# translearn/PaintRL

Measured on NVIDIA B200. Metric: batched env steps/sec, higher is better.
Workload: dtype f64

## Files before the change

### paintrl_b200/csrc/paintrl_kernels.cuh

```cuda
#pragma once
#include "paintrl_device.cuh"

namespace paintrl {

struct StepIO {
    const void *actions;
    double *obs, *reward, *penalty, *actual;
    uint8_t *done;
    int32_t *new_texels;
    double *next_obs;
    const int32_t *reset_start_idx;
};

struct EnvSel {
    const int32_t *ids;
    int lo, n;
};

template <bool SUBSET>
__device__ __forceinline__ bool step_env(const EnvSel &sel, int k, int num_envs, int &env) {
    if (!SUBSET) { env = k; return k < num_envs; }
    if (k >= sel.n) return false;
    env = sel.ids ? __ldg(&sel.ids[k]) : sel.lo + k;
    return (unsigned)env < (unsigned)num_envs;
}

struct EnvArrays {
    EnvState *states;
    MoveOut *moves;
    EnvStat *env_stats;
    unsigned *bits;
    int16_t *thick;
    unsigned *grid_cnt;
    unsigned *ready;
    ShotPoses *shots;
    unsigned *last_mask;
};

constexpr int kStageWords = 512;

template <bool STAGED>
struct alignas(128) WarpScratch {
    unsigned sbits[STAGED ? kStageWords : 32];
    EnvState st;
    MoveOut mv;
    int rowL[kMaxRows], rowU[kMaxRows];
    int rowWa[kMaxRows], rowWn[kMaxRows];
    uint16_t cand[STAGED ? kStageWords : 2];
    double hsi_r[2 * kPaintPerAction];
    unsigned long long bar;
};
static_assert(2 * kMaxRows >= 2 * kMaxObs, "the section histogram aliases rowWa / rowWn");

template <bool STAGED>
struct Bits {
    unsigned *g;
    unsigned *s;
    __device__ __forceinline__ unsigned ld(int w) const { return STAGED ? s[w] : __ldcg(g + w); }
    __device__ __forceinline__ void st(int w, unsigned v) const {
        if (STAGED) s[w] = v; else __stcg(g + w, v);
    }
};

__device__ __forceinline__ unsigned smem_addr(const void *p) { return (unsigned)__cvta_generic_to_shared(p); }
__device__ __forceinline__ void mbar_init(unsigned long long *bar, int count) {
    asm volatile("mbarrier.init.shared::cta.b64 [%0], %1;" ::"r"(smem_addr(bar)), "r"(count) : "memory");
    asm volatile("fence.proxy.async.shared::cta;" ::: "memory");
}
__device__ __forceinline__ void mbar_expect_tx(unsigned long long *bar, unsigned bytes) {
    asm volatile("mbarrier.arrive.expect_tx.shared::cta.b64 _, [%0], %1;" ::"r"(smem_addr(bar)), "r"(bytes) : "memory");
}
__device__ __forceinline__ void bulk_g2s(void *dst, const void *src, unsigned bytes, unsigned long long *bar) {
    asm volatile("cp.async.bulk.shared::cluster.global.mbarrier::complete_tx::bytes [%0], [%1], %2, [%3];" ::"r"(smem_addr(dst)),
                 "l"(src), "r"(bytes), "r"(smem_addr(bar))
                 : "memory");
}
__device__ __forceinline__ void mbar_wait(unsigned long long *bar, unsigned phase) {
    asm volatile(
        "{\n"
        ".reg .pred p;\n"
        "WAIT_%=:\n"
        "mbarrier.try_wait.parity.shared::cta.b64 p, [%0], %1;\n"
        "@p bra DONE_%=;\n"
        "bra WAIT_%=;\n"
        "DONE_%=:\n"
        "}" ::"r"(smem_addr(bar)), "r"(phase)
        : "memory");
}
__device__ __forceinline__ void bulk_s2g(void *dst, const void *src, unsigned bytes) {
    asm volatile("cp.async.bulk.global.shared::cta.bulk_group [%0], [%1], %2;" ::"l"(dst), "r"(smem_addr(src)), "r"(bytes)
                 : "memory");
    asm volatile("cp.async.bulk.commit_group;" ::: "memory");
}
__device__ __forceinline__ void bulk_wait_read() { asm volatile("cp.async.bulk.wait_group.read 0;" ::: "memory"); }
__device__ __forceinline__ void fence_async_smem() { asm volatile("fence.proxy.async.shared::cta;" ::: "memory"); }

__device__ __forceinline__ unsigned lowmask(int n) {
    unsigned m;
    asm("bmsk.clamp.b32 %0, 0, %1;" : "=r"(m) : "r"(n));
    return m;
}
__device__ __forceinline__ int clamp32(int v) { return max(v, 0); }

__device__ __forceinline__ unsigned *bits_of(const DevPack &pk, const EnvArrays &ea, int env) {
    return ea.bits + (size_t)env * pk.n_words_pad;
}
__device__ __forceinline__ int16_t *thick_of(const DevPack &pk, const EnvArrays &ea, int env) {
    return ea.thick ? ea.thick + (size_t)env * pk.n_slots : nullptr;
}
__device__ __forceinline__ unsigned *grid_cnt_of(const DevPack &pk, const EnvArrays &ea, int env) {
    return ea.grid_cnt ? ea.grid_cnt + (size_t)env * pk.n_gcells_pad : nullptr;
}
__device__ __forceinline__ const double *axis_table(const DevPack &pk, int a) {
    return a == 0 ? pk.tx : (a == 1 ? pk.ty : pk.tz);
}

template <typename WS>
__device__ __forceinline__ void row_ranks(const DevPack &pk, const Ax &ax, double p0, int lane, WS &ws) {
    const double f = floor((p0 - pk.cx_o0) * pk.cx_inv);
    const double *kx = axis_table(pk, ax.a0);
    for (int r = lane; r < pk.n_rows; r += 32) {
        const int n = __ldg(&pk.row_count[r]);
        int L, U;
        if (!(f >= 0.0)) {
            L = U = 0;
        } else if (f >= (double)pk.ncx) {
            L = U = n;
        } else {
// ... 228 lines not shown
    const double2 *src = reinterpret_cast<const double2 *>(&st);
    double2 v = src[0];
#pragma unroll
    for (int i = 1; i < 8; ++i) if (lane == i) v = src[i];
    if (lane < 8) reinterpret_cast<double2 *>(g)[lane] = v;
}

__device__ __forceinline__ int auto_start_index(const DevPack &pk, const DevConfig &cfg, int env, int episode) {
    return (int)(splitmix64(cfg.seed ^ splitmix64(((unsigned long long)env << 32) | (unsigned)episode)) %
                 (unsigned long long)pk.n_starts);
}

constexpr float kBallEps = 1e-7f;
constexpr int NS = kPaintPerAction;

struct ShotsF { float x[NS + 1], y[NS + 1], z[NS + 1]; };

template <typename WS>
__device__ __forceinline__ double cen(const WS &ws, int s, int k) {
    return s < NS ? ws.mv.centers[s][k] : ws.st.last_center[k];
}

__device__ __forceinline__ bool ball_pretest_at(const ShotsF &c, float tx, float ty, float tz, float e[NS + 1]) {
    const float nr2f = -(float)(kPaintRadius * kPaintRadius);
    float m = INFINITY;
#pragma unroll
    for (int s = 0; s <= NS; ++s) {
        const float dx = tx - c.x[s], dy = ty - c.y[s], dz = tz - c.z[s];
        e[s] = fmaf(dz, dz, fmaf(dy, dy, fmaf(dx, dx, nr2f)));
        m = fminf(m, fabsf(e[s]));
    }
    return m <= kBallEps;
}
__device__ __forceinline__ bool ball_pretest(const DevPack &pk, const ShotsF &c, int j, float e[NS + 1]) {
    return ball_pretest_at(c, __ldg(&pk.fx[j]), __ldg(&pk.fy[j]), __ldg(&pk.fz[j]), e);
}

template <typename WS>
__device__ __forceinline__ bool ball_exact(const WS &ws, double x, double y, double z, int s) {
    const double r2 = kPaintRadius * kPaintRadius;
    const double dx = x - cen(ws, s, 0), dy = y - cen(ws, s, 1), dz = z - cen(ws, s, 2);
    return (dx * dx + dy * dy + dz * dz) <= r2;
}

template <typename WS>
__device__ __forceinline__ unsigned ball_mask(const DevPack &pk, const ShotsF &c, const WS &ws, int j, bool has_last) {
    float e[NS + 1];
    unsigned in = 0;
    if (ball_pretest(pk, c, j, e)) {
        const double x = __ldg(&pk.tx[j]), y = __ldg(&pk.ty[j]), z = __ldg(&pk.tz[j]);
#pragma unroll
        for (int s = 0; s <= NS; ++s) in |= (ball_exact(ws, x, y, z, s) ? 1u : 0u) << s;
    } else {
#pragma unroll
        for (int s = 0; s <= NS; ++s) in |= (e[s] <= 0.f ? 1u : 0u) << s;
    }
    if (!has_last) in &= (1u << NS) - 1u;
    return in;
}

template <typename WS>
__device__ __forceinline__ void ball_flags_at(const DevPack &pk, const ShotsF &c, const WS &ws, int j, float tx, float ty, float tz,
                                              bool has_last, bool &any_shot, bool &possible) {
    float e[NS + 1];
    bool in[NS + 1];
    if (ball_pretest_at(c, tx, ty, tz, e)) {
        const double x = __ldg(&pk.tx[j]), y = __ldg(&pk.ty[j]), z = __ldg(&pk.tz[j]);
#pragma unroll
        for (int s = 0; s <= NS; ++s) in[s] = ball_exact(ws, x, y, z, s);
    } else {
#pragma unroll
        for (int s = 0; s <= NS; ++s) in[s] = e[s] <= 0.f;
    }
    bool prev = has_last && in[NS];
    any_shot = false;
    possible = false;
#pragma unroll
    for (int s = 0; s < NS; ++s) {
        any_shot = any_shot || in[s];
        possible = possible || (in[s] && !prev);
        prev = in[s];
    }
}
template <typename WS>
__device__ __forceinline__ void ball_flags(const DevPack &pk, const ShotsF &c, const WS &ws, int j, bool has_last, bool &any_shot,
                                           bool &possible) {
    ball_flags_at(pk, c, ws, j, __ldg(&pk.fx[j]), __ldg(&pk.fy[j]), __ldg(&pk.fz[j]), has_last, any_shot, possible);
}

template <bool STAGED, int COLOR, typename WS>
__device__ __forceinline__ int stamp_ranges(const DevPack &pk, float lo0, float hi0, float lo1, float hi1, int lane, WS &ws) {
    const float rr = (float)kPaintRadius + 4e-5f;
    int base = 0;
    for (int r0 = 0; r0 < pk.n_rows; r0 += 32) {
        const int r = r0 + lane;
        int wa = 0, wn = 0;
        if (r < pk.n_rows) {
            const float ylo = fmaf((float)r, pk.rel_row_h, pk.rel_row_o1) - 2e-5f, yhi = ylo + pk.rel_row_h + 4e-5f;
            const float dy = fmaxf(0.f, fmaxf(ylo - hi1, lo1 - yhi));
            if (dy <= rr) {
                const float hw = sqrtf(rr * rr - dy * dy) + 4e-5f;
                const float fa = floorf((lo0 - hw - pk.rel_cx_o0) * pk.rel_cx_inv) - 1.f;
                const float fb = floorf((hi0 + hw - pk.rel_cx_o0) * pk.rel_cx_inv) + 1.f;
                if (fb >= 0.f && fa < (float)pk.ncx) {
                    const int ca = (int)fmaxf(fa, 0.f), cb = (int)fminf(fb, (float)(pk.ncx - 1));
                    const int *cs = pk.cell_start + (size_t)r * (pk.ncx + 1);
                    const int i0 = __ldg(cs + ca), i1 = __ldg(cs + cb + 1);
                    if (i1 > i0) {
                        wa = __ldg(&pk.row_word0[r]) + (i0 >> 5);
                        wn = ((i1 - 1) >> 5) - (i0 >> 5) + 1;
                    }
                }
            }
            ws.rowWa[r] = wa;
            ws.rowWn[r] = wn;
        }
        if (STAGED) {
            int incl = wn;
#pragma unroll
            for (int o = 1; o < 32; o <<= 1) {
                const int u = __shfl_up_sync(kFull, incl, o);
                if (lane >= o) incl += u;
            }
            const int at = base + incl - wn;
            for (int t = 0; t < wn; ++t) ws.cand[at + t] = (uint16_t)(wa + t);
            base += __shfl_sync(kFull, incl, 31);
        }
    }
    __syncwarp();
    return base;
}

template <bool STAGED, typename WS, typename BodyFn>
__device__ __forceinline__ void for_each_stamp_word(const DevPack &pk, int lane, const WS &ws, int n_cand, BodyFn body) {
    if constexpr (STAGED) {
        for (int k = 0; k < n_cand; ++k) body((int)ws.cand[k]);
    } else {
        for (int r0 = 0; r0 < pk.n_rows; r0 += 32) {
            const int r = r0 + lane;
            const int wa = r < pk.n_rows ? ws.rowWa[r] : 0, wn = r < pk.n_rows ? ws.rowWn[r] : 0;
            unsigned m = __ballot_sync(kFull, wn > 0);
            while (m) {
                const int src = __ffs(m) - 1;
                m &= m - 1;
                const int a = __shfl_sync(kFull, wa, src), n = __shfl_sync(kFull, wn, src);
                for (int w = a; w < a + n; ++w) body(w);
            }
        }
    }
}

template <int COLOR, bool STAGED, typename WS, typename BITS>
__device__ __forceinline__ void stamp(const DevPack &pk, const Ax &ax, const BITS &bits, int16_t *thick, unsigned *grid_cnt, bool has_last,
                                      int lane, WS &ws, int &n_new_out, int &n_possible_out, bool &dirty_out PAINTRL_PROF_PARAM) {
    ShotsF c;
#pragma unroll
    for (int s = 0; s <= NS; ++s) {
        c.x[s] = (float)(cen(ws, s, 0) - pk.org0);
        c.y[s] = (float)(cen(ws, s, 1) - pk.org1);
        c.z[s] = (float)(cen(ws, s, 2) - pk.org2);
    }
    float lo0 = INFINITY, hi0 = -INFINITY, lo1 = INFINITY, hi1 = -INFINITY;
#pragma unroll
    for (int s = 0; s < NS; ++s) {
        const float c0 = ax.a0 == 0 ? c.x[s] : (ax.a0 == 1 ? c.y[s] : c.z[s]);
        const float c1 = ax.a1 == 0 ? c.x[s] : (ax.a1 == 1 ? c.y[s] : c.z[s]);
        lo0 = fminf(lo0, c0); hi0 = fmaxf(hi0, c0);
        lo1 = fminf(lo1, c1); hi1 = fmaxf(hi1, c1);
    }
    PAINTRL_PROF(17, lane == 0);
    const int n_cand = stamp_ranges<STAGED, COLOR>(pk, lo0, hi0, lo1, hi1, lane, ws);
    PAINTRL_PROF(18, lane == 0);

    double rmax[NS];
    if (COLOR == 1) {
#pragma unroll
        for (int s = 0; s < NS; ++s) rmax[s] = -1.0;
        for_each_stamp_word<STAGED>(pk, lane, ws, n_cand, [&](int w) {
            const int j = w * 32 + lane;
            const unsigned in = ball_mask(pk, c, ws, j, false);
            if (in) {
                const double x = __ldg(&pk.tx[j]), y = __ldg(&pk.ty[j]), z = __ldg(&pk.tz[j]);
#pragma unroll
                for (int s = 0; s < NS; ++s) {
                    if (in & (1u << s)) {
                        const double dx = x - cen(ws, s, 0), dy = y - cen(ws, s, 1), dz = z - cen(ws, s, 2);
                        rmax[s] = fmax(rmax[s], dx * dx + dy * dy + dz * dz);
                    }
                }
            }
        });
#pragma unroll
        for (int s = 0; s < NS; ++s) rmax[s] = sqrt(warp_max(rmax[s]));
        if (lane < NS) {
            double r = rmax[0];
#pragma unroll
            for (int s = 1; s < NS; ++s) r = lane == s ? rmax[s] : r;
            ws.hsi_r[lane] = r;
            ws.hsi_r[NS + lane] = r > 0.0 ? 1.0 / (r * r) : 0.0;
        }
        __syncwarp();
    }

    int n_new = 0, n_possible = 0;
    unsigned any = 0;
    if (COLOR == 0 && !STAGED) {
        constexpr int kBatch = 4;
        for (int r0 = 0; r0 < pk.n_rows; r0 += 32) {
            const int r = r0 + lane;
            const int wa = r < pk.n_rows ? ws.rowWa[r] : 0, wn = r < pk.n_rows ? ws.rowWn[r] : 0;
            unsigned m = __ballot_sync(kFull, wn > 0);
            while (m) {
                const int src = __ffs(m) - 1;
// ... 1 lines not shown
                const int a = __shfl_sync(kFull, wa, src), n = __shfl_sync(kFull, wn, src);
                for (int w0 = a; w0 < a + n; w0 += kBatch) {
                    float tx[kBatch], ty[kBatch], tz[kBatch];
                    unsigned old[kBatch];
#pragma unroll
                    for (int q = 0; q < kBatch; ++q) {
                        const int w = min(w0 + q, a + n - 1);
                        const int j = w * 32 + lane;
                        tx[q] = __ldg(&pk.fx[j]); ty[q] = __ldg(&pk.fy[j]); tz[q] = __ldg(&pk.fz[j]);
                        old[q] = bits.ld(w);
                    }
#pragma unroll
                    for (int q = 0; q < kBatch; ++q) {
                        const int w = w0 + q;
                        if (w >= a + n) break;
                        const int j = w * 32 + lane;
                        bool any_shot, possible;
                        ball_flags_at(pk, c, ws, j, tx[q], ty[q], tz[q], has_last, any_shot, possible);
                        const unsigned uni = __ballot_sync(kFull, any_shot);
                        if (uni == 0u) continue;
                        n_possible += __popc(__ballot_sync(kFull, possible));
                        const unsigned flipped = uni & ~old[q];
                        if (flipped) {
                            n_new += __popc(flipped);
                            if (lane == 0) bits.st(w, old[q] | uni);
                            any |= flipped;
                            if (grid_cnt && ((flipped >> lane) & 1u)) atomicAdd(grid_cnt + __ldg(&pk.gcell[j]), 1u);
                        }
                    }
                }
            }
        }
    } else if (COLOR == 0) {
        for_each_stamp_word<STAGED>(pk, lane, ws, n_cand, [&](int w) {
            const int j = w * 32 + lane;
            bool any_shot, possible;
            ball_flags(pk, c, ws, j, has_last, any_shot, possible);
            const unsigned uni = __ballot_sync(kFull, any_shot);
            if (uni == 0u) return;
            n_possible += __popc(__ballot_sync(kFull, possible));
            const unsigned old = bits.ld(w);
            __syncwarp();
            const unsigned flipped = uni & ~old;
            if (flipped) {
                n_new += __popc(flipped);
                if (lane == 0) bits.st(w, old | uni);
                any |= flipped;
                if (grid_cnt && ((flipped >> lane) & 1u)) atomicAdd(grid_cnt + __ldg(&pk.gcell[j]), 1u);
            }
        });
    } else {
        for_each_stamp_word<STAGED>(pk, lane, ws, n_cand, [&](int w) {
            const int j = w * 32 + lane;
            const unsigned in = ball_mask(pk, c, ws, j, has_last);
            const unsigned shots = in & ((1u << NS) - 1u);
            const unsigned uni = __ballot_sync(kFull, shots != 0u);
            if (uni == 0u) return;
            const unsigned prev = ((shots << 1) | (in >> NS)) & ((1u << NS) - 1u);
            n_possible += __popc(__ballot_sync(kFull, (shots & ~prev) != 0u));
            bool fl = false;
            if (shots) {
                const int sv0 = (int)__ldcg(&thick[j]);
                int sv = sv0;
                const double x = __ldg(&pk.tx[j]), y = __ldg(&pk.ty[j]), z = __ldg(&pk.tz[j]);
#pragma unroll 1
                for (int s = 0; s < NS; ++s) {
                    if ((shots & (1u << s)) && sv > 0) {
                        const double dx = x - cen(ws, s, 0), dy = y - cen(ws, s, 1), dz = z - cen(ws, s, 2);
                        const double d2 = dx * dx + dy * dy + dz * dz;
                        const double qa = kHsiTargetMax * (1.0 - d2 * ws.hsi_r[NS + s]);
                        const double qf = floor(qa);
                        int quantity = (int)qf + 1;
                        if (!(qa > 1e-9 && qa - qf > 1e-9 && (qf + 1.0) - qa > 1e-9)) {
                            const double ratio = sqrt(d2) / ws.hsi_r[s];
                            quantity = (int)(kHsiTargetMax * (1.0 - ratio * ratio)) + 1;
                        }
                        sv -= quantity;
                        n_new += quantity;
                    }
                }
                if (sv != sv0) {
                    __stcg(&thick[j], (int16_t)sv);
                    fl = (sv0 == kPainted);
                }
            }
            const unsigned flipped = __ballot_sync(kFull, fl);
            if (flipped) {
// ... 488 lines not shown
        }
        r = slab_pass<G>(blob + 4, n_planes, frm, d0, d1, d2, grp);
        if (r.outside || r.t_in > r.t_out || r.t_in > 1.0 || r.t_out < 0.0) return 0;
        candidate = false;
        if (!(r.t_in > -INFINITY)) { if (link != 0ull) continue; why = 3; break; }
        candidate = true;
        h.x = frm.x + d0 * r.t_in; h.y = frm.y + d1 * r.t_in; h.z = frm.z + d2 * r.t_in;
        if (in_cell_region_idx(pk, comp(h, ax.a0), comp(h, ax.a1), comp(h, npax), cell, abv, clv, hpv)) {
            if (!(0.0 <= r.t_in)) return 0;
            if (n_verts <= 0) { PAINTRL_FAST_REASON(5); return 2; }
            ref.blob = blob; ref.n_planes = n_planes; ref.n_verts = n_verts;
            hit = h;
            return 1;
        }
    }
    path_counts += 1 << 8;
    if (pair_proves_miss(pk, *miss_cache_ptr, r, candidate, frm, d0, d1, d2)) return 0;
    if (candidate) {
        path_counts += 1 << 16;
        if (near_violations_rolled<G>(reinterpret_cast<const double2 *>(pk.planes), pk.n_planes, h, grp) ==
            near_violations_rolled<G>(sub, n_sub, h, grp)) {
            if (!(r.t_in <= r.t_out && 0.0 <= r.t_in && r.t_in <= 1.0)) return 0;
            ref.blob = nullptr;
            hit = h;
            return 1;
        }
        why = 6;
    }
    PAINTRL_FAST_REASON(why);
    (void)why;
    return 2;
}

template <int G, bool AX12, bool DISCRETE, bool FUSED>
__device__ __forceinline__ bool move_fast_body(const DevPack &pk, const DevConfig &cfg, const EnvArrays &ea, int env, int row, const void *actions,
                                               EnvState *sst, MoveOut *smv) {
    const Ax ax = make_ax<AX12>(pk.axis0, pk.axis1);
    const int lane = threadIdx.x & 31;
    const Grp grp = make_grp<G>(lane);
    PAINTRL_TRACE_MARK(env, 0, grp.gl == 0);
    PAINTRL_TRACE_SM(env, 6, grp.gl == 0);
    EnvState *gst = FUSED ? sst : &ea.states[env];
    Vec3 cur_p, cur_n;
    double last_angle;
    int term_counter = gst->term_counter, flags = gst->flags;
    {
        const double2 s0 = reinterpret_cast<const double2 *>(gst)[0], s1 = reinterpret_cast<const double2 *>(gst)[1],
                      s2 = reinterpret_cast<const double2 *>(gst)[2];
        const double q[4] = {s1.y, s2.x, s2.y, gst->quat[3]};
        last_angle = gst->last_angle;
        cur_p.x = s0.x; cur_p.y = s0.y; cur_p.z = s1.x;
        cur_n = tcp_orn_norm(cur_p, q);
    }
    double u1, u2, new_angle;
    if (DISCRETE) {
        const long long a = reinterpret_cast<const long long *>(actions)[row];
        const int ai = (int)min(max(a, 0ll), (long long)cfg.discrete_granularity);
        u1 = __ldg(&cfg.discrete_table[3 * ai]);
        u2 = __ldg(&cfg.discrete_table[3 * ai + 1]);
        new_angle = __ldg(&cfg.discrete_table[3 * ai + 2]);
    } else {
        const double *a = reinterpret_cast<const double *>(actions) + (size_t)row * cfg.action_shape;
        double a0 = a[0];
        if (!(-1.0 <= a0 && a0 <= 1.0)) a0 = a0 < -1.0 ? -1.0 : 1.0;
        if (cfg.action_shape == 1) {
            const double phi = (a0 + 1.0) * kPi;
            u1 = cos(phi);
            u2 = sin(phi);
        } else {
            double a1v = a[1];
            if (!(-1.0 <= a1v && a1v <= 1.0)) a1v = a1v < -1.0 ? -1.0 : 1.0;
            const double phi = atan2(a1v, a0);
            const double x = fabs(a0), y = fabs(a1v);
            if (x == 0.0 && y == 0.0) { u1 = x; u2 = y; }
            else { const double m = fmax(x, y); u1 = m * cos(phi); u2 = m * sin(phi); }
        }
        const double da1 = u1 * kStepSize, da2 = u2 * kStepSize;
        new_angle = (da1 != 0.0) ? atan(fabs(da2 / da1)) : kPi / 2;
    }
    const double delta1 = (u1 * kStepSize) / kPaintPerAction, delta2 = (u2 * kStepSize) / kPaintPerAction;
    const int counter_before = term_counter;
    int path_counts = 0, path_sizes = 0;
    double quat[4];
    MoveOut *mv = FUSED ? smv : &ea.moves[env];
    double *centers = &mv->centers[0][0];
#pragma unroll 1
    for (int s = 0; s < kPaintPerAction; ++s) {
        const double delta2_scaled = delta2 * pk.lwr;
        Vec3 p = cur_p;
        add_comp(p, ax.a0, delta1);
        add_comp(p, ax.a1, delta2_scaled);
        const Vec3 end = {p.x + cur_n.x, p.y + cur_n.y, p.z + cur_n.z};
        Vec3 hit, pos, center;
        CellRef ref;
        double2 vc0 = make_double2(0.0, 0.0), vc1 = vc0;
        const double *rec = nullptr;
        const int code = ray_fast<G>(pk, ax, p, end, grp, hit, ref, vc0, vc1, delta1, delta2_scaled, s + 1 < kPaintPerAction,
                                     &ea.moves[env].miss_cache, path_counts, path_sizes);
        if (code == 2) {
            if (!FUSED && grp.gl == 0)
                asm volatile("st.release.gpu.global.u32 [%0], %1;" ::"l"(ea.ready + env), "r"(kReadyBailed) : "memory");
            PAINTRL_TRACE_MARK(env, 1, grp.gl == 0);
            return true;
// ... 30 lines not shown
    if (grp.gl == 0 && env < 65536) g_trace[env][6] |= ((unsigned long long)(unsigned)path_counts << 16) | ((unsigned long long)(unsigned)path_sizes << 48);
#endif
    (void)path_sizes;
    if (FUSED) __syncwarp();
    if (grp.gl == 0) {
        reinterpret_cast<double2 *>(gst)[0] = make_double2(cur_p.x, cur_p.y);
        reinterpret_cast<double2 *>(gst)[1] = make_double2(cur_p.z, quat[0]);
        reinterpret_cast<double2 *>(gst)[2] = make_double2(quat[1], quat[2]);
        gst->quat[3] = quat[3];
        reinterpret_cast<double2 *>(&gst->last_angle)[0] = make_double2(new_angle, fabs(new_angle - last_angle));
        gst->term_counter = term_counter;
        gst->flags = flags;
        mv->counts = term_counter - counter_before;
        if (!FUSED) asm volatile("st.release.gpu.global.u32 [%0], %1;" ::"l"(ea.ready + env), "r"(kReadyMoved) : "memory");
    }
    PAINTRL_TRACE_MARK(env, 1, grp.gl == 0);
    return false;
}

#ifndef PAINTRL_MOVE_FAST_MINB
#define PAINTRL_MOVE_FAST_MINB 7
#endif
template <int G, bool AX12, bool DISCRETE, bool SUBSET = false>
__global__ void __launch_bounds__(kWarpsPerBlock * 32, PAINTRL_MOVE_FAST_MINB)
move_fast_kernel(DevPack pk, DevConfig cfg, EnvArrays ea, int num_envs, const void *actions, EnvSel sel) {
    asm volatile("griddepcontrol.launch_dependents;");
    const int k = (blockIdx.x * blockDim.x + threadIdx.x) / G;
    int env;
    if (!step_env<SUBSET>(sel, k, num_envs, env)) return;
    if (cfg.debug_bail_mod > 0 && env % cfg.debug_bail_mod == 0) {
        if ((threadIdx.x & (G - 1)) == 0) asm volatile("st.release.gpu.global.u32 [%0], %1;" ::"l"(ea.ready + env), "r"(kReadyBailed) : "memory");
        return;
    }
    move_fast_body<G, AX12, DISCRETE, false>(pk, cfg, ea, env, k, actions, nullptr, nullptr);
}

struct ColdArgs { DevPack pk; DevConfig cfg; EnvArrays ea; };
__device__ __noinline__ void move_generic_cold(const ColdArgs *ca, int env, int row, const void *actions) {
    move_body<32, false>(ca->pk, ca->cfg, ca->ea, env, row, actions);
}

template <int COLOR, bool STAGED, bool AX12, bool FUSED = false, bool DISCRETE = false, bool NORMAL = false>
__device__ __forceinline__ void paint_body(const DevPack &pk, const DevConfig &cfg, const EnvArrays &ea, int env, int row, const StepIO &io,
                                           WarpScratch<STAGED> &ws, const ColdArgs *cold, NormalScratch *ns = nullptr) {
    const Ax ax = make_ax<AX12>(pk.axis0, pk.axis1);
    typedef WarpScratch<STAGED> WS;
    const int lane = threadIdx.x & 31;
    PAINTRL_PROF_BEGIN(env, 15, 32)
    PAINTRL_TRACE_MARK(env, 2, lane == 0);
    PAINTRL_TRACE_SM(env, 7, lane == 0);
    unsigned *gbits = bits_of(pk, ea, env), *grid_cnt = grid_cnt_of(pk, ea, env);
    int16_t *thick = thick_of(pk, ea, env);
    const unsigned plane_bytes = (unsigned)pk.n_words_pad * 4u;
    if (STAGED && lane == 0) {
        mbar_init(&ws.bar, 1);
        mbar_expect_tx(&ws.bar, plane_bytes);
        bulk_g2s(ws.sbits, gbits, plane_bytes, &ws.bar);
    }
    int bailed = 0;
    if (FUSED) {
        if (lane < 8) reinterpret_cast<double2 *>(&ws.st)[lane] = __ldcg(reinterpret_cast<const double2 *>(&ea.states[env]) + lane);
        __syncwarp();
        if (cfg.debug_bail_mod > 0 && env % cfg.debug_bail_mod == 0) bailed = 1;
        else bailed = move_fast_body<32, AX12, DISCRETE, true>(pk, cfg, ea, env, row, io.actions, &ws.st, &ws.mv) ? 1 : 0;
        __syncwarp();
    } else {
        if (lane == 0) {
            const unsigned *flag = ea.ready + env;
            unsigned v;
            for (;;) {
                asm volatile("ld.acquire.gpu.global.u32 %0, [%1];" : "=r"(v) : "l"(flag) : "memory");
                if (v != 0u) break;
                __nanosleep(200);
            }
            ea.ready[env] = 0u;
            bailed = (v == kReadyBailed);
        }
        bailed = __shfl_sync(kFull, bailed, 0);
    }
    if (bailed) {
        move_generic_cold(cold, env, row, io.actions);
        __threadfence();
        if (lane == 0) ea.ready[env] = 0u;
    }
    __syncwarp();
    PAINTRL_TRACE_MARK(env, 3, lane == 0);
    if (!FUSED || bailed) {
        if (lane < 16) {
            const double2 *src = lane < 8 ? reinterpret_cast<const double2 *>(&ea.states[env]) + lane
                                          : reinterpret_cast<const double2 *>(&ea.moves[env]) + (lane - 8);
            double2 *dst = lane < 8 ? reinterpret_cast<double2 *>(&ws.st) + lane : reinterpret_cast<double2 *>(&ws.mv) + (lane - 8);
            *dst = __ldcg(src);
        }
        __syncwarp();
    }
    if (STAGED) mbar_wait(&ws.bar, 0);
    PAINTRL_TRACE_MARK(env, 4, lane == 0);
    PAINTRL_PROF(16, lane == 0);
    const Bits<STAGED> bits = {gbits, ws.sbits};
    EnvState &st = ws.st;
    const Vec3 cur_p = {st.pose[0], st.pose[1], st.pose[2]};
    const bool fast4 = (cfg.obs_mode == 0 || cfg.obs_mode == 3) && cfg.obs_grad == 4;
    if (fast4) {
        row_ranks(pk, ax, comp(cur_p, ax.a0), lane, ws);
        const int prow = pose_row(pk, comp(cur_p, ax.a1));
        if (prow >= 0 && prow < pk.n_rows) {
            const int w0 = __ldg(&pk.row_word0[prow]), w1 = __ldg(&pk.row_word0[prow + 1]);
            const char *ky = reinterpret_cast<const char *>(axis_table(pk, ax.a1) + (size_t)w0 * 32);
            for (int k = lane; k < 2 * (w1 - w0); k += 32) prefetch_l1(ky + (size_t)k * 128);
        }
    }
    PAINTRL_PROF(15, lane == 0);

    const bool has_last = (st.flags & kFlagHasLast) != 0;
    int n_new, n_possible;
    bool dirty;
    if (NORMAL) {
        const double *src = reinterpret_cast<const double *>(&ea.shots[env]);
        for (int i = lane; i < kPaintPerAction * 7; i += 32) (&ns->pos[0][0])[i] = __ldcg(src + i);
        __syncwarp();
        stamp_normal<COLOR>(pk, cfg, ax, bits, thick, grid_cnt, ea.last_mask + (size_t)env * pk.n_words_pad, lane, ws, *ns, n_new, n_possible, dirty);
    } else {
        stamp<COLOR, STAGED>(pk, ax, bits, thick, grid_cnt, has_last, lane, ws, n_new, n_possible, dirty PAINTRL_PROF_PASS);
    }
    PAINTRL_PROF(19, lane == 0);

    int flags = st.flags | kFlagHasLast;
    const double succeeded = (COLOR == 0) ? (double)n_new : (double)n_new / 255.0;
    if ((ws.mv.counts & 0xf) >= kPaintPerAction && n_possible == 0) flags |= kFlagTerminate;
    const double radius = kPaintRadius;
    const double axis1_real = comp(cur_p, ax.a0), axis2_real = comp(cur_p, ax.a1);
    double rate, reward, turn, axis2_in, rel;
    {
        double num = succeeded, den = n_possible ? (double)n_possible : 1.0;
        if (lane == 1) den = 100.0;
        if (lane == 2) { num = st.angle_diff; den = kPi; }
        if (lane == 3) { num = axis2_real - pk.range1_min + radius; den = pk.range1_max - pk.range1_min + 2 * radius; }
        if (lane == 4) { num = axis2_real - pk.range1_min; den = pk.range1_max - pk.range1_min; }
        double q = 0.0;
        if (num != 0.0) q = num / den;
        rate = n_possible ? __shfl_sync(kFull, q, 0) : 0.0;
        reward = __shfl_sync(kFull, q, 1);
        turn = __shfl_sync(kFull, q, 2);
        axis2_in = __shfl_sync(kFull, q, 3);
        rel = __shfl_sync(kFull, q, 4);
    }
    const double total_reward = st.total_reward + reward;
    double penalty = 0.2;
    if (cfg.overlap_penalty) penalty += 0.1 * (1 - rate);
    if (cfg.turning_penalty) penalty += 0.1 * turn;
    const double actual = reward - penalty;
    const int step_counter = st.step_counter + 1;
    int gi;
    {
        const double scaled = rel * pk.grid_granularity;
        gi = !(scaled > -1.0) ? 0 : (scaled >= (double)pk.grid_granularity ? pk.grid_granularity - 1 : (int)scaled);
// ... 90 lines not shown
        if (next_obs) {
            const double *src = pk.reset_obs + (size_t)idx * cfg.obs_dim;
            for (int i = lane; i < cfg.obs_dim; i += 32) next_obs[i] = __ldg(&src[i]);
        }
    } else if (STAGED && dirty) {
        fence_async_smem();
        __syncwarp();
        if (lane == 0) bulk_s2g(gbits, ws.sbits, plane_bytes);
    }
    __syncwarp();
    if (lane < 8) reinterpret_cast<double2 *>(&ea.states[env])[lane] = reinterpret_cast<const double2 *>(&st)[lane];
    if (STAGED && lane == 0) bulk_wait_read();
    PAINTRL_PROF(26, lane == 0);
    PAINTRL_TRACE_MARK(env, 5, lane == 0);
}

#ifndef PAINTRL_PAINT_OCC
#define PAINTRL_PAINT_OCC 28
#endif
template <int COLOR, bool STAGED, bool AX12, int WPB, bool SUBSET = false>
__global__ void __launch_bounds__(WPB * 32, (STAGED ? PAINTRL_PAINT_OCC : 16) / WPB)
paint_kernel(DevPack pk, DevConfig cfg, EnvArrays ea, int num_envs, StepIO io, const ColdArgs *cold, EnvSel sel) {
    __shared__ WarpScratch<STAGED> scratch[WPB];
    const int warp = threadIdx.x >> 5;
    const int k = blockIdx.x * WPB + warp;
    int env;
    if (!step_env<SUBSET>(sel, k, num_envs, env)) return;
    paint_body<COLOR, STAGED, AX12>(pk, cfg, ea, env, k, io, scratch[warp], cold);
}

template <int COLOR, bool SUBSET = false>
__global__ void __launch_bounds__(32, 14)
paint_normal_kernel(DevPack pk, DevConfig cfg, EnvArrays ea, int num_envs, StepIO io, const ColdArgs *cold, EnvSel sel) {
    __shared__ WarpScratch<true> scratch[1];
    __shared__ NormalScratch nscratch[1];
    const int k = blockIdx.x;
    int env;
    if (!step_env<SUBSET>(sel, k, num_envs, env)) return;
    paint_body<COLOR, true, false, false, false, true>(pk, cfg, ea, env, k, io, scratch[0], cold, &nscratch[0]);
}

#ifndef PAINTRL_FUSED_WPB
#define PAINTRL_FUSED_WPB 1
#endif
template <int COLOR, bool STAGED, bool AX12, bool DISCRETE, bool SUBSET = false>
__global__ void __launch_bounds__(32 * PAINTRL_FUSED_WPB, (STAGED ? PAINTRL_PAINT_OCC : 16) / PAINTRL_FUSED_WPB)
step_fused_kernel(DevPack pk, DevConfig cfg, EnvArrays ea, int num_envs, StepIO io, const ColdArgs *cold, EnvSel sel) {
    __shared__ WarpScratch<STAGED> scratch[PAINTRL_FUSED_WPB];
    const int warp = threadIdx.x >> 5;
    const int k = blockIdx.x * PAINTRL_FUSED_WPB + warp;
    int env;
    if (!step_env<SUBSET>(sel, k, num_envs, env)) return;
    l2_prefetch_tables(pk, blockIdx.x * blockDim.x + threadIdx.x, gridDim.x * blockDim.x);
    paint_body<COLOR, STAGED, AX12, true, DISCRETE>(pk, cfg, ea, env, k, io, scratch[warp], cold);
}

__global__ void __launch_bounds__(kWarpsPerBlock * 32)
reset_kernel(DevPack pk, DevConfig cfg, EnvArrays ea, int num_envs, const int32_t *env_ids, int n, const int32_t *start_idx,
             const double *set_pos, const double *set_normal, double *obs_out, int mode ) {
    const Ax ax = make_ax<false>(pk.axis0, pk.axis1);
    __shared__ WarpScratch<false> scratch[kWarpsPerBlock];
    const int lane = threadIdx.x & 31, warp = threadIdx.x >> 5;
    const int k = blockIdx.x * kWarpsPerBlock + warp;
    if (k >= n) return;
    const int env = env_ids ? env_ids[k] : k;
    if ((unsigned)env >= (unsigned)num_envs) return;
    unsigned *gbits = bits_of(pk, ea, env), *grid_cnt = grid_cnt_of(pk, ea, env);
// ... 146 lines not shown
```

### profiles/phase_profile.py

```python
#!/usr/bin/env python
import argparse, ctypes, os, sys
sys.path.insert(0, os.path.dirname(os.path.dirname(os.path.abspath(__file__))))
import torch
import bench
from paintrl_b200 import _capi
from paintrl_b200.batched_env import BatchedPaintEnv
from paintrl_b200.config import EnvConfig

NAMES = {0: 'move: load + action + first p', 1: 'move: p / end of later sub-steps', 6: 'ray: guess cell, entry, issue blob loads',
         7: 'ray: slab pass (div, reductions)', 8: 'ray: region check / accept', 9: 'ray: verify / full scan / hit',
         10: 'hook: nearest vertex', 11: 'hook: triangles + pick', 12: 'move: pose, quat, centre', 13: 'move: stores',
         15: 'paint: early row ranks + TCP-row prefetch', 16: 'paint: TMA loads + mbarrier wait', 17: 'stamp: shot floats, bbox', 18: 'stamp: row ranges', 19: 'stamp: words (ball tests, bits)',
         20: 'score + termination', 21: 'obs: normalised pose', 22: 'obs: row ranks', 23: 'obs: rows + words (popc)',
         24: 'obs: TCP row', 25: 'obs: reductions + write', 26: 'paint: outputs, reset, stores'}

ap = argparse.ArgumentParser()
ap.add_argument('--envs', type=int, default=4096)
ap.add_argument('--workload', default='c2')
ap.add_argument('--steps', type=int, default=50)
ap.add_argument('--no-flush', action='store_true')
ap.add_argument('--per-env', action='store_true', help='last step: phase cycles of the slowest move warps and by slow-path class')
ap.add_argument('--dump-rays', default=None, help='write the rays that left the fast path to this .npy file')
args = ap.parse_args()
w = bench.WORKLOADS[args.workload]
cfg = EnvConfig(w['extra'], auto_reset=True, seed=1234, **w['kw'])
dev = torch.device('cuda:0')
env = BatchedPaintEnv(args.envs, cfg, device=dev)
lib = _capi.lib()
lib.paintrl_debug_profile.restype = ctypes.c_int
lib.paintrl_debug_profile.argtypes = [ctypes.c_void_p, ctypes.c_int]
gen = torch.Generator(device=dev); gen.manual_seed(1234)
acts = torch.randint(0, cfg.discrete_granularity, (args.steps + 10, args.envs), generator=gen, device=dev, dtype=torch.int64)
env.reset(torch.randint(0, env.n_starts, (args.envs,), generator=gen, device=dev, dtype=torch.int32))
flush = torch.empty(512 << 20, dtype=torch.uint8, device=dev)
for i in range(10):
    env.step(acts[i])
buf = (ctypes.c_ulonglong * 64)()
if lib.paintrl_debug_profile(buf, 1) == 0:
    raise SystemExit('not an instrumented build: PAINTRL_PROFILE=1 python -m paintrl_b200.build --force')
for i in range(args.steps):
    if not args.no_flush:
        flush.fill_(i & 255)
    env.step(acts[10 + i])
lib.paintrl_debug_profile(buf, 0)
if args.dump_rays:
# ... 34 lines not shown
```

Baseline: 77.68 million.

## Prefetch stamp coordinates via cp.async ring and fuse row ranks into stamp ranges

In the staged stamp loop, a 4-deep shared-memory ring is filled with cp.async so the float coordinates of upcoming candidate words load ahead of the ball tests, hiding global load latency. Row rank computation is merged into the stamp_ranges per-row pass, so the cell_start reads are shared and a separate row_ranks sweep is avoided on the non-normal path. The action load is hoisted so it overlaps the state load in the fused path. The cost is more shared memory per warp and more unconditional loads in stamp_ranges.

```diff
diff --git a/paintrl_b200/csrc/paintrl_kernels.cuh b/paintrl_b200/csrc/paintrl_kernels.cuh
--- a/paintrl_b200/csrc/paintrl_kernels.cuh
+++ b/paintrl_b200/csrc/paintrl_kernels.cuh
@@ -39,7 +39,10 @@
 
 constexpr int kStageWords = 512;
 
-template <bool STAGED>
+constexpr int kCoordRing = 4;
+static_assert((kCoordRing & (kCoordRing - 1)) == 0, "the ring slot is k % kCoordRing");
+
+template <bool STAGED, bool RING = STAGED>
 struct alignas(128) WarpScratch {
     unsigned sbits[STAGED ? kStageWords : 32];
     EnvState st;
@@ -47,6 +50,7 @@
     int rowL[kMaxRows], rowU[kMaxRows];
     int rowWa[kMaxRows], rowWn[kMaxRows];
     uint16_t cand[STAGED ? kStageWords : 2];
+    float ring[RING ? kCoordRing * 96 : 1];
     double hsi_r[2 * kPaintPerAction];
     unsigned long long bar;
 };
@@ -94,6 +98,13 @@
 }
 __device__ __forceinline__ void bulk_wait_read() { asm volatile("cp.async.bulk.wait_group.read 0;" ::: "memory"); }
 __device__ __forceinline__ void fence_async_smem() { asm volatile("fence.proxy.async.shared::cta;" ::: "memory"); }
+
+__device__ __forceinline__ void cp_async4(void *dst, const void *src) {
+    asm volatile("cp.async.ca.shared.global [%0], [%1], 4;" ::"r"(smem_addr(dst)), "l"(src) : "memory");
+}
+__device__ __forceinline__ void cp_async_commit() { asm volatile("cp.async.commit_group;" ::: "memory"); }
+template <int N>
+__device__ __forceinline__ void cp_async_wait() { asm volatile("cp.async.wait_group %0;" ::"n"(N) : "memory"); }
 
 __device__ __forceinline__ unsigned lowmask(int n) {
     unsigned m;
@@ -388,9 +399,6 @@
     }
     return m <= kBallEps;
 }
-__device__ __forceinline__ bool ball_pretest(const DevPack &pk, const ShotsF &c, int j, float e[NS + 1]) {
-    return ball_pretest_at(c, __ldg(&pk.fx[j]), __ldg(&pk.fy[j]), __ldg(&pk.fz[j]), e);
-}
 
 template <typename WS>
 __device__ __forceinline__ bool ball_exact(const WS &ws, double x, double y, double z, int s) {
@@ -400,10 +408,11 @@
 }
 
 template <typename WS>
-__device__ __forceinline__ unsigned ball_mask(const DevPack &pk, const ShotsF &c, const WS &ws, int j, bool has_last) {
+__device__ __forceinline__ unsigned ball_mask(const DevPack &pk, const ShotsF &c, const WS &ws, int j, float tx, float ty, float tz,
+                                              bool has_last) {
     float e[NS + 1];
     unsigned in = 0;
-    if (ball_pretest(pk, c, j, e)) {
+    if (ball_pretest_at(c, tx, ty, tz, e)) {
         const double x = __ldg(&pk.tx[j]), y = __ldg(&pk.ty[j]), z = __ldg(&pk.tz[j]);
 #pragma unroll
         for (int s = 0; s <= NS; ++s) in |= (ball_exact(ws, x, y, z, s) ? 1u : 0u) << s;
@@ -438,38 +447,66 @@
         prev = in[s];
     }
 }
-template <typename WS>
-__device__ __forceinline__ void ball_flags(const DevPack &pk, const ShotsF &c, const WS &ws, int j, bool has_last, bool &any_shot,
-                                           bool &possible) {
-    ball_flags_at(pk, c, ws, j, __ldg(&pk.fx[j]), __ldg(&pk.fy[j]), __ldg(&pk.fz[j]), has_last, any_shot, possible);
-}
 
 template <bool STAGED, int COLOR, typename WS>
-__device__ __forceinline__ int stamp_ranges(const DevPack &pk, float lo0, float hi0, float lo1, float hi1, int lane, WS &ws) {
+__device__ __forceinline__ int stamp_ranges(const DevPack &pk, const Ax &ax, float lo0, float hi0, float lo1, float hi1, bool ranks, double p0,
+                                            int lane, WS &ws) {
     const float rr = (float)kPaintRadius + 4e-5f;
+    const double f = ranks ? floor((p0 - pk.cx_o0) * pk.cx_inv) : -1.0;
+    const bool f_in = f >= 0.0 && f < (double)pk.ncx;
+    const int fc = f_in ? (int)f : 0;
+    const double *kx = axis_table(pk, ax.a0);
     int base = 0;
     for (int r0 = 0; r0 < pk.n_rows; r0 += 32) {
         const int r = r0 + lane;
         int wa = 0, wn = 0;
         if (r < pk.n_rows) {
+            const int *cs = pk.cell_start + (size_t)r * (pk.ncx + 1);
             const float ylo = fmaf((float)r, pk.rel_row_h, pk.rel_row_o1) - 2e-5f, yhi = ylo + pk.rel_row_h + 4e-5f;
             const float dy = fmaxf(0.f, fmaxf(ylo - hi1, lo1 - yhi));
+            bool hit = false;
+            int ca = 0, cb = 0;
             if (dy <= rr) {
                 const float hw = sqrtf(rr * rr - dy * dy) + 4e-5f;
                 const float fa = floorf((lo0 - hw - pk.rel_cx_o0) * pk.rel_cx_inv) - 1.f;
                 const float fb = floorf((hi0 + hw - pk.rel_cx_o0) * pk.rel_cx_inv) + 1.f;
                 if (fb >= 0.f && fa < (float)pk.ncx) {
-                    const int ca = (int)fmaxf(fa, 0.f), cb = (int)fminf(fb, (float)(pk.ncx - 1));
-                    const int *cs = pk.cell_start + (size_t)r * (pk.ncx + 1);
-                    const int i0 = __ldg(cs + ca), i1 = __ldg(cs + cb + 1);
-                    if (i1 > i0) {
-                        wa = __ldg(&pk.row_word0[r]) + (i0 >> 5);
-                        wn = ((i1 - 1) >> 5) - (i0 >> 5) + 1;
+                    hit = true;
+                    ca = (int)fmaxf(fa, 0.f);
+                    cb = (int)fminf(fb, (float)(pk.ncx - 1));
+                }
+            }
+            const int i0 = __ldg(cs + ca), i1 = __ldg(cs + cb + 1), w0 = __ldg(&pk.row_word0[r]);
+            const int k0 = ranks ? __ldg(cs + fc) : 0, k1 = ranks ? __ldg(cs + fc + 1) : 0, n = ranks ? __ldg(&pk.row_count[r]) : 0;
+            if (hit && i1 > i0) {
+                wa = w0 + (i0 >> 5);
+                wn = ((i1 - 1) >> 5) - (i0 >> 5) + 1;
+            }
+            ws.rowWa[r] = wa;
+            ws.rowWn[r] = wn;
+            if (ranks) {
+                int L, U;
+                if (!(f >= 0.0)) {
+                    L = U = 0;
+                } else if (!f_in) {
+                    L = U = n;
+                } else {
+                    const double *k = kx + (size_t)w0 * 32 + k0;
+                    const double x0 = __ldg(k), x1 = __ldg(k + 1), x2 = __ldg(k + 2), x3 = __ldg(k + 3);
+                    const int c = k1 - k0;
+                    L = k0 + ((c > 0 && x0 < p0) ? 1 : 0) + ((c > 1 && x1 < p0) ? 1 : 0) + ((c > 2 && x2 < p0) ? 1 : 0) +
+                        ((c > 3 && x3 < p0) ? 1 : 0);
+                    U = k0 + ((c > 0 && x0 <= p0) ? 1 : 0) + ((c > 1 && x1 <= p0) ? 1 : 0) + ((c > 2 && x2 <= p0) ? 1 : 0) +
+                        ((c > 3 && x3 <= p0) ? 1 : 0);
+                    for (int i = 4; i < c; ++i) {
+                        const double x = __ldg(&k[i]);
+                        L += (x < p0) ? 1 : 0;
+                        U += (x <= p0) ? 1 : 0;
                     }
                 }
-            }
-            ws.rowWa[r] = wa;
-            ws.rowWn[r] = wn;
+                ws.rowL[r] = L;
+                ws.rowU[r] = U;
+            }
         }
         if (STAGED) {
             int incl = wn;
@@ -488,9 +525,27 @@
 }
 
 template <bool STAGED, typename WS, typename BodyFn>
-__device__ __forceinline__ void for_each_stamp_word(const DevPack &pk, int lane, const WS &ws, int n_cand, BodyFn body) {
+__device__ __forceinline__ void for_each_stamp_word(const DevPack &pk, int lane, WS &ws, int n_cand, BodyFn body) {
     if constexpr (STAGED) {
-        for (int k = 0; k < n_cand; ++k) body((int)ws.cand[k]);
+        auto issue = [&](int k, int slot) {
+            if (k < n_cand) {
+                const int j = (int)ws.cand[k] * 32 + lane;
+                cp_async4(&ws.ring[slot * 96 + lane], pk.fx + j);
+                cp_async4(&ws.ring[slot * 96 + 32 + lane], pk.fy + j);
+                cp_async4(&ws.ring[slot * 96 + 64 + lane], pk.fz + j);
+            }
+            cp_async_commit();
+        };
+#pragma unroll
+        for (int k = 0; k < kCoordRing; ++k) issue(k, k);
+        for (int k = 0; k < n_cand; ++k) {
+            const int slot = k % kCoordRing;
+            cp_async_wait<kCoordRing - 1>();
+            const float *r = &ws.ring[slot * 96 + lane];
+            const float tx = r[0], ty = r[32], tz = r[64];
+            issue(k + kCoordRing, slot);
+            body((int)ws.cand[k], tx, ty, tz);
+        }
     } else {
         for (int r0 = 0; r0 < pk.n_rows; r0 += 32) {
             const int r = r0 + lane;
@@ -500,7 +555,10 @@
                 const int src = __ffs(m) - 1;
                 m &= m - 1;
                 const int a = __shfl_sync(kFull, wa, src), n = __shfl_sync(kFull, wn, src);
-                for (int w = a; w < a + n; ++w) body(w);
+                for (int w = a; w < a + n; ++w) {
+                    const int j = w * 32 + lane;
+                    body(w, __ldg(&pk.fx[j]), __ldg(&pk.fy[j]), __ldg(&pk.fz[j]));
+                }
             }
         }
     }
@@ -508,7 +566,8 @@
 
 template <int COLOR, bool STAGED, typename WS, typename BITS>
 __device__ __forceinline__ void stamp(const DevPack &pk, const Ax &ax, const BITS &bits, int16_t *thick, unsigned *grid_cnt, bool has_last,
-                                      int lane, WS &ws, int &n_new_out, int &n_possible_out, bool &dirty_out PAINTRL_PROF_PARAM) {
+                                      bool ranks, double p0, int lane, WS &ws, int &n_new_out, int &n_possible_out,
+                                      bool &dirty_out PAINTRL_PROF_PARAM) {
     ShotsF c;
 #pragma unroll
     for (int s = 0; s <= NS; ++s) {
@@ -525,16 +584,16 @@
         lo1 = fminf(lo1, c1); hi1 = fmaxf(hi1, c1);
     }
     PAINTRL_PROF(17, lane == 0);
-    const int n_cand = stamp_ranges<STAGED, COLOR>(pk, lo0, hi0, lo1, hi1, lane, ws);
+    const int n_cand = stamp_ranges<STAGED, COLOR>(pk, ax, lo0, hi0, lo1, hi1, ranks, p0, lane, ws);
     PAINTRL_PROF(18, lane == 0);
 
     double rmax[NS];
     if (COLOR == 1) {
 #pragma unroll
         for (int s = 0; s < NS; ++s) rmax[s] = -1.0;
-        for_each_stamp_word<STAGED>(pk, lane, ws, n_cand, [&](int w) {
+        for_each_stamp_word<STAGED>(pk, lane, ws, n_cand, [&](int w, float tx, float ty, float tz) {
             const int j = w * 32 + lane;
-            const unsigned in = ball_mask(pk, c, ws, j, false);
+            const unsigned in = ball_mask(pk, c, ws, j, tx, ty, tz, false);
             if (in) {
                 const double x = __ldg(&pk.tx[j]), y = __ldg(&pk.ty[j]), z = __ldg(&pk.tz[j]);
 #pragma unroll
@@ -602,10 +661,10 @@
             }
         }
     } else if (COLOR == 0) {
-        for_each_stamp_word<STAGED>(pk, lane, ws, n_cand, [&](int w) {
+        for_each_stamp_word<STAGED>(pk, lane, ws, n_cand, [&](int w, float tx, float ty, float tz) {
             const int j = w * 32 + lane;
             bool any_shot, possible;
-            ball_flags(pk, c, ws, j, has_last, any_shot, possible);
+            ball_flags_at(pk, c, ws, j, tx, ty, tz, has_last, any_shot, possible);
             const unsigned uni = __ballot_sync(kFull, any_shot);
             if (uni == 0u) return;
             n_possible += __popc(__ballot_sync(kFull, possible));
@@ -620,9 +679,9 @@
             }
         });
     } else {
-        for_each_stamp_word<STAGED>(pk, lane, ws, n_cand, [&](int w) {
+        for_each_stamp_word<STAGED>(pk, lane, ws, n_cand, [&](int w, float tx, float ty, float tz) {
             const int j = w * 32 + lane;
-            const unsigned in = ball_mask(pk, c, ws, j, has_last);
+            const unsigned in = ball_mask(pk, c, ws, j, tx, ty, tz, has_last);
             const unsigned shots = in & ((1u << NS) - 1u);
             const unsigned uni = __ballot_sync(kFull, shots != 0u);
             if (uni == 0u) return;
@@ -1177,8 +1236,27 @@
     return 2;
 }
 
+struct ActionIn { double v0, v1, v2; };
+template <bool DISCRETE>
+__device__ __forceinline__ ActionIn load_action(const DevConfig &cfg, const void *actions, int row) {
+    ActionIn in;
+    if (DISCRETE) {
+        const long long a = reinterpret_cast<const long long *>(actions)[row];
+        const int ai = (int)min(max(a, 0ll), (long long)cfg.discrete_granularity);
+        in.v0 = __ldg(&cfg.discrete_table[3 * ai]);
+        in.v1 = __ldg(&cfg.discrete_table[3 * ai + 1]);
+        in.v2 = __ldg(&cfg.discrete_table[3 * ai + 2]);
+    } else {
+        const double *a = reinterpret_cast<const double *>(actions) + (size_t)row * cfg.action_shape;
+        in.v0 = a[0];
+        in.v1 = cfg.action_shape == 1 ? 0.0 : a[1];
+        in.v2 = 0.0;
+    }
+    return in;
+}
+
 template <int G, bool AX12, bool DISCRETE, bool FUSED>
-__device__ __forceinline__ bool move_fast_body(const DevPack &pk, const DevConfig &cfg, const EnvArrays &ea, int env, int row, const void *actions,
+__device__ __forceinline__ bool move_fast_body(const DevPack &pk, const DevConfig &cfg, const EnvArrays &ea, int env, const ActionIn act,
                                                EnvState *sst, MoveOut *smv) {
     const Ax ax = make_ax<AX12>(pk.axis0, pk.axis1);
     const int lane = threadIdx.x & 31;
@@ -1199,21 +1277,18 @@
     }
     double u1, u2, new_angle;
     if (DISCRETE) {
-        const long long a = reinterpret_cast<const long long *>(actions)[row];
-        const int ai = (int)min(max(a, 0ll), (long long)cfg.discrete_granularity);
-        u1 = __ldg(&cfg.discrete_table[3 * ai]);
-        u2 = __ldg(&cfg.discrete_table[3 * ai + 1]);
-        new_angle = __ldg(&cfg.discrete_table[3 * ai + 2]);
+        u1 = act.v0;
+        u2 = act.v1;
+        new_angle = act.v2;
     } else {
-        const double *a = reinterpret_cast<const double *>(actions) + (size_t)row * cfg.action_shape;
-        double a0 = a[0];
+        double a0 = act.v0;
         if (!(-1.0 <= a0 && a0 <= 1.0)) a0 = a0 < -1.0 ? -1.0 : 1.0;
         if (cfg.action_shape == 1) {
             const double phi = (a0 + 1.0) * kPi;
             u1 = cos(phi);
             u2 = sin(phi);
         } else {
-            double a1v = a[1];
+            double a1v = act.v1;
             if (!(-1.0 <= a1v && a1v <= 1.0)) a1v = a1v < -1.0 ? -1.0 : 1.0;
             const double phi = atan2(a1v, a0);
             const double x = fabs(a0), y = fabs(a1v);
@@ -1310,7 +1385,7 @@
         if ((threadIdx.x & (G - 1)) == 0) asm volatile("st.release.gpu.global.u32 [%0], %1;" ::"l"(ea.ready + env), "r"(kReadyBailed) : "memory");
         return;
     }
-    move_fast_body<G, AX12, DISCRETE, false>(pk, cfg, ea, env, k, actions, nullptr, nullptr);
+    move_fast_body<G, AX12, DISCRETE, false>(pk, cfg, ea, env, load_action<DISCRETE>(cfg, actions, k), nullptr, nullptr);
 }
 
 struct ColdArgs { DevPack pk; DevConfig cfg; EnvArrays ea; };
@@ -1320,9 +1395,9 @@
 
 template <int COLOR, bool STAGED, bool AX12, bool FUSED = false, bool DISCRETE = false, bool NORMAL = false>
 __device__ __forceinline__ void paint_body(const DevPack &pk, const DevConfig &cfg, const EnvArrays &ea, int env, int row, const StepIO &io,
-                                           WarpScratch<STAGED> &ws, const ColdArgs *cold, NormalScratch *ns = nullptr) {
+                                           WarpScratch<STAGED, STAGED && !NORMAL> &ws, const ColdArgs *cold, NormalScratch *ns = nullptr) {
     const Ax ax = make_ax<AX12>(pk.axis0, pk.axis1);
-    typedef WarpScratch<STAGED> WS;
+    typedef WarpScratch<STAGED, STAGED && !NORMAL> WS;
     const int lane = threadIdx.x & 31;
     PAINTRL_PROF_BEGIN(env, 15, 32)
     PAINTRL_TRACE_MARK(env, 2, lane == 0);
@@ -1337,10 +1412,13 @@
     }
     int bailed = 0;
     if (FUSED) {
-        if (lane < 8) reinterpret_cast<double2 *>(&ws.st)[lane] = __ldcg(reinterpret_cast<const double2 *>(&ea.states[env]) + lane);
+        double2 rec;
+        if (lane < 8) rec = __ldcg(reinterpret_cast<const double2 *>(&ea.states[env]) + lane);
+        const ActionIn act = load_action<DISCRETE>(cfg, io.actions, row);
+        if (lane < 8) reinterpret_cast<double2 *>(&ws.st)[lane] = rec;
         __syncwarp();
         if (cfg.debug_bail_mod > 0 && env % cfg.debug_bail_mod == 0) bailed = 1;
-        else bailed = move_fast_body<32, AX12, DISCRETE, true>(pk, cfg, ea, env, row, io.actions, &ws.st, &ws.mv) ? 1 : 0;
+        else bailed = move_fast_body<32, AX12, DISCRETE, true>(pk, cfg, ea, env, act, &ws.st, &ws.mv) ? 1 : 0;
         __syncwarp();
     } else {
         if (lane == 0) {
@@ -1380,7 +1458,7 @@
     const Vec3 cur_p = {st.pose[0], st.pose[1], st.pose[2]};
     const bool fast4 = (cfg.obs_mode == 0 || cfg.obs_mode == 3) && cfg.obs_grad == 4;
     if (fast4) {
-        row_ranks(pk, ax, comp(cur_p, ax.a0), lane, ws);
+        if (NORMAL) row_ranks(pk, ax, comp(cur_p, ax.a0), lane, ws);
         const int prow = pose_row(pk, comp(cur_p, ax.a1));
         if (prow >= 0 && prow < pk.n_rows) {
             const int w0 = __ldg(&pk.row_word0[prow]), w1 = __ldg(&pk.row_word0[prow + 1]);
@@ -1393,13 +1471,14 @@
     const bool has_last = (st.flags & kFlagHasLast) != 0;
     int n_new, n_possible;
     bool dirty;
-    if (NORMAL) {
+    if constexpr (NORMAL) {
         const double *src = reinterpret_cast<const double *>(&ea.shots[env]);
         for (int i = lane; i < kPaintPerAction * 7; i += 32) (&ns->pos[0][0])[i] = __ldcg(src + i);
         __syncwarp();
         stamp_normal<COLOR>(pk, cfg, ax, bits, thick, grid_cnt, ea.last_mask + (size_t)env * pk.n_words_pad, lane, ws, *ns, n_new, n_possible, dirty);
     } else {
-        stamp<COLOR, STAGED>(pk, ax, bits, thick, grid_cnt, has_last, lane, ws, n_new, n_possible, dirty PAINTRL_PROF_PASS);
+        stamp<COLOR, STAGED>(pk, ax, bits, thick, grid_cnt, has_last, fast4, comp(cur_p, ax.a0), lane, ws, n_new, n_possible,
+                             dirty PAINTRL_PROF_PASS);
     }
     PAINTRL_PROF(19, lane == 0);
 
@@ -1556,7 +1635,7 @@
 template <int COLOR, bool SUBSET = false>
 __global__ void __launch_bounds__(32, 14)
 paint_normal_kernel(DevPack pk, DevConfig cfg, EnvArrays ea, int num_envs, StepIO io, const ColdArgs *cold, EnvSel sel) {
-    __shared__ WarpScratch<true> scratch[1];
+    __shared__ WarpScratch<true, false> scratch[1];
     __shared__ NormalScratch nscratch[1];
     const int k = blockIdx.x;
     int env;
diff --git a/profiles/phase_profile.py b/profiles/phase_profile.py
--- a/profiles/phase_profile.py
+++ b/profiles/phase_profile.py
@@ -10,7 +10,7 @@
 NAMES = {0: 'move: load + action + first p', 1: 'move: p / end of later sub-steps', 6: 'ray: guess cell, entry, issue blob loads',
          7: 'ray: slab pass (div, reductions)', 8: 'ray: region check / accept', 9: 'ray: verify / full scan / hit',
          10: 'hook: nearest vertex', 11: 'hook: triangles + pick', 12: 'move: pose, quat, centre', 13: 'move: stores',
-         15: 'paint: early row ranks + TCP-row prefetch', 16: 'paint: TMA loads + mbarrier wait', 17: 'stamp: shot floats, bbox', 18: 'stamp: row ranges', 19: 'stamp: words (ball tests, bits)',
+         15: 'paint: TCP-row prefetch (normal method: + row ranks)', 16: 'paint: TMA loads + mbarrier wait', 17: 'stamp: shot floats, bbox', 18: 'stamp: row ranges (+ row ranks)', 19: 'stamp: words (ball tests, bits)',
          20: 'score + termination', 21: 'obs: normalised pose', 22: 'obs: row ranks', 23: 'obs: rows + words (popc)',
          24: 'obs: TCP row', 25: 'obs: reductions + write', 26: 'paint: outputs, reset, stores'}
 
```

After: 76.89 million (median of 6 runs). -1.0%, worse.
